# qradiolink/qradiolink

Measured on AMD Instinct MI355X. Metric: IQ MSamples/sec through RX demod chain, higher is better.
Workload: dtype f32

## Files before the change

### qradiolink_amd/csrc/engine.cpp

```cpp
#include "demod.hpp"
#include <cmath>
#include <cstdlib>
#include <memory>
#include <new>

#ifndef QRL_FEC_GATE_US
#define QRL_FEC_GATE_US 30u
#endif
#ifndef QRL_DEV_SKIP
#define QRL_DEV_SKIP 0
#endif

int qrl_demod::flush_fec(bool behind_front_end)
{
    if (!fec_deferred) return QRL_OK;
    fec_deferred = false;
    HIPCHK(hipStreamWaitEvent(fecs, ev_q[fec_pending_slot], 0));
    if (behind_front_end) {
        HIPCHK(hipStreamWaitEvent(fecs, ev_ff, 0));
        launch_fec_gate(QRL_FEC_GATE_US, fecs);
    }
    launch_fec(fec_pending, cfg.batch, fecs);
    HIPCHK(hipEventRecord(ev_fec[fec_pending_slot], fecs));
    return QRL_OK;
// ... 235 lines not shown
        if ((r = fll_lo.upload(to_f2(lo))) || (r = fll_up.upload(to_f2(up)))) return r;
        control_loop_gains((float)(8 * M_PI / 100), fll_alpha, fll_beta);
        fll_maxf = (float)(2 * M_PI * (2.0 / sps_eff));
        if ((r = fll_st.alloc(B))) return r;
        if ((r = tanh_tab.upload(tanh_table())) || (r = qp_st.alloc(B))) return r;
        control_loop_gains((float)(2 * M_PI / 200), c2_alpha, c2_beta);
    } else if (fam == F_QPSK) {
        if ((r = tanh_tab.upload(tanh_table())) || (r = qp_st.alloc(B))) return r;
        control_loop_gains((float)(M_PI / 200 / sps_eff), c1_alpha, c1_beta);
        control_loop_gains((float)(qpsk_fll ? M_PI / 200 : M_PI / 400), c2_alpha, c2_beta);
        if (qpsk_fll) {
            std::vector<std::complex<float>> lo, up;
            fll_band_edge_taps((float)sps_eff, 0.35f, 32, lo, up);
            if ((r = fll_lo.upload(to_f2(lo))) || (r = fll_up.upload(to_f2(up)))) return r;
            control_loop_gains((float)(2 * M_PI / 100), fll_alpha, fll_beta);
            fll_maxf = (float)(2 * M_PI * (2.0 / sps_eff));
            if ((r = fll_st.alloc(B))) return r;
        }
        const float symbol_rate = (float)target / (float)sps_eff;
        const float dev = 200.0f / symbol_rate;
        clock_loop_gains((float)(2 * M_PI / (symbol_rate / 10)), 1.0f, 0.2869f, ss_alpha, ss_beta);
        ss_maxp = (float)sps_eff + dev; ss_minp = (float)sps_eff - dev;
        const float ang = (float)(-3 * M_PI / 4);
        qp_rot = make_float2((float)std::cos((double)ang), (float)std::sin((double)ang));
    } else {
        const std::vector<float> sf = low_pass(1, target, target / sps_eff, target / sps_eff, WIN_HAMMING);
        symf_nt = (int)sf.size();
        if ((r = symf_taps.upload(sf))) return r;
        demod_gain = (float)(sps_eff / (M_PI / 2));
        clock_loop_gains((float)(2 * M_PI / 200.0f), 1.0f, 0.2869f, ss_alpha, ss_beta);
        ss_maxp = (float)sps_eff + 0.05f; ss_minp = (float)sps_eff - 0.05f;
    }
    if ((r = ss_st.alloc(B)) || (r = fec_st.alloc((size_t)B * 2)) || (r = counts_scratch.alloc((size_t)B * 4))) return r;
    if (loops_family() && (r = qp_snap.alloc((size_t)B * 2))) return r;
    if ((fam == F_ANALOG && (r = an.build(*this, mx.n2))) || (fam == F_DSSS && (r = ds.build(*this, mx.n2)))) return r;
    return init_state();
}

int qrl_demod::process(const void* iq, size_t stride, size_t n, const qrl_demod_out* out, int fmt)
{
    if (fmt == IN_SC16 && !fe.used)
        return qrl_set_error(QRL_ERR_ARG, "qrl_demod_process_sc16: int16 input needs the device-rate front end (device_samp_rate >= 2000000); this handle runs at 1 Msps");
    if (n > cfg.max_chunk) return qrl_set_error(QRL_ERR_TOO_BIG, "n exceeds max_chunk");
    if (fmt == IN_SC16) {
        if (!sc16_rows_ok("qrl_demod_process_sc16", iq, stride)) return QRL_ERR_ARG;
    } else if ((reinterpret_cast<uintptr_t>(iq) & 15u) || (stride & 1u)) return qrl_set_error(QRL_ERR_ARG, "iq must be 16-byte aligned, stride even");
    const int B = cfg.batch;
    uint32_t* counts = (out && out->counts) ? out->counts : counts_scratch.p;
    hipStream_t cs = overlap ? tail : stream;
    const int slot = (int)(call_no & 1);
    if (overlap) {
        if (tail2_valid[slot]) HIPCHK(hipStreamWaitEvent(stream, ev_tail2[slot], 0));
    } else {
        HIPCHK(hipMemsetAsync(counts, 0, (size_t)B * 4 * sizeof(uint32_t), stream));
    }
    if (loops_family() && q_valid[slot]) HIPCHK(hipStreamWaitEvent(stream, ev_q[slot], 0));
    if (grouped && q_valid[slot ^ 1]) HIPCHK(hipStreamWaitEvent(stream, ev_q[slot ^ 1], 0));
    if (pre_pending) { HIPCHK(hipStreamWaitEvent(stream, ev_pre, 0)); pre_pending = false; }
    const bool use_pre = pre && input_resident;
    const float2* in = reinterpret_cast<const float2*>(iq);
    const float2* hist_old = hist_flip ? hist_b.p : hist_a.p;
    const PortC fport = filtered_port(out), cport = constellation_port(out);
    float2* hist_new = hist_flip ? hist_a.p : hist_b.p;

    const uint64_t n_in0 = n_in, n_in1 = n_in + n;
    uint64_t n1_0 = n1, n1_1 = n1;
    RingC r2{s2.p, s2_mask}, r2l{s2l.p, s2_mask}, r2f{s2f.p, s2_mask};
    RingF r2d{s2d.p, s2_mask}, r3{s3.p, s2_mask};

    hipEvent_t ev0 = nullptr, ev1 = nullptr;
    if (profiling) {
        HIPCHK(hipEventCreate(&ev0)); HIPCHK(hipEventCreate(&ev1));
        HIPCHK(hipEventRecord(ev0, stream));
    }
    if (fe.used) {
        n1_1 = decim_count(n_in1, 1, fe_decim);
        DecimParams p{};
        p.in = in; p.in_stride = stride; p.n0 = n_in0; p.n = (uint32_t)n;
        p.hist = hist_old; p.hist_len = hist_len;
        p.out = RingC{s1.p, s1_mask}; p.m0 = n1_0; p.m_count = (uint32_t)(n1_1 - n1_0);
        p.taps = fe.taps.p; p.D = fe.D; p.Jpad = fe.c.Jpad;
        p.rot_enable = 1; rot.fill(p);
        p.in_fmt = fmt; p.in_scale = sc16_scale;
        if (use_pre) { p.pre_stream = pre; p.pre_event = ev_pre; }
        if (fe.launch(p, B, stream, use_pre ? slot : 0)) return qrl_set_error(QRL_ERR_HIP, "front-end launch: hipFuncSetAttribute failed");
    }
    if (profiling && fe.used) { HIPCHK(hipEventRecord(ev1, stream)); prof_events.emplace_back(ev0, ev1); }
    const uint64_t src0 = fe.used ? n1_0 : n_in0, src1 = fe.used ? n1_1 : n_in1;
    const uint64_t n2_0 = n2, n2_1 = decim_count(src1, interp, decim);
    if (interp == 1) {
        DecimParams p{};
        input_source(p, in, stride, hist_old, src0, src1);
        p.out = r2; p.m0 = n2_0; p.m_count = (uint32_t)(n2_1 - n2_0);
        p.taps = first.taps.p; p.D = first.D; p.Jpad = first.c.Jpad;
        if (d2f) {
            Dec2FirParams f{};
            f.d = p; f.taps = d2f_taps.p; f.out = RingC{s2f.p, s2_mask};
            f.port = fport.p; f.port_cap = fport.cap; f.counts = counts;
            launch_dec2_fir(f, B, stream);
        } else {
            if (use_pre && !fe.used) { p.pre_stream = pre; p.pre_event = ev_pre; }
            if (first.launch(p, B, stream, use_pre && !fe.used ? slot : 0)) return qrl_set_error(QRL_ERR_HIP, "first-stage launch: hipFuncSetAttribute failed");
        }
    } else {
        ResampParams p{};
        input_source(p, in, stride, hist_old, src0, src1);
        p.out = r2; p.q0 = n2_0; p.q_count = (uint32_t)(n2_1 - n2_0);
        p.taps = rs_taps.p; p.I = interp; p.D = decim; p.Jp = rs_Jp;
        if (fam == F_DMR && !m17) {
            p.port = fport.p; p.port_cap = fport.cap; p.port_counts = counts;
        }
        launch_resamp(p, B, stream);
    }
    if (profiling && !fe.used) { HIPCHK(hipEventRecord(ev1, stream)); prof_events.emplace_back(ev0, ev1); }
    if (scope_out) {
        const uint64_t ns_1 = decim_count(src1, 1, scope_D);
        DecimParams p{};
        input_source(p, in, stride, hist_old, src0, src1);
        p.out = RingC{s_scope.p, scope_mask}; p.m0 = n_scope; p.m_count = (uint32_t)(ns_1 - n_scope);
        p.taps = scope.taps.p; p.D = scope.D; p.Jpad = scope.c.Jpad;
        if (scope.launch(p, B, stream)) return qrl_set_error(QRL_ERR_HIP, "scope launch: hipFuncSetAttribute failed");
        launch_ring_store(RingC{s_scope.p, scope_mask}, n_scope, (uint32_t)(ns_1 - n_scope), scope_out, scope_cap, scope_counts, B, stream);
        n_scope = ns_1;
    }
    {
        HistParams h{};
        h.in = in; h.in_stride = stride; h.n0 = n_in0; h.n = (uint32_t)n;
        h.hist_old = hist_old; h.hist_new = hist_new; h.hist_len = hist_len;
        h.rot_enable = 1; rot.fill(h);
        h.in_fmt = fmt; h.in_scale = sc16_scale;
        if (pre) { HIPCHK(hipEventRecord(ev_fe[slot], stream)); fe_valid[slot] = true; }
        if (use_pre) {
            if (fe_valid[slot ^ 1]) HIPCHK(hipStreamWaitEvent(pre, ev_fe[slot ^ 1], 0));
            launch_hist_save(h, B, pre);
            HIPCHK(hipEventRecord(ev_pre, pre));
            pre_pending = true;
        } else launch_hist_save(h, B, stream);
        hist_flip = !hist_flip;
    }
    if (overlap) {
        HIPCHK(hipEventRecord(ev_ff, stream));
        HIPCHK(hipStreamWaitEvent(tail, ev_ff, 0));
        HIPCHK(hipMemsetAsync(counts, 0, (size_t)B * 4 * sizeof(uint32_t), tail));
    }
    const uint32_t c2 = (uint32_t)(n2_1 - n2_0);
    if (fam == F_DSSS || fam == F_ANALOG) {
        if (int rr = fam == F_DSSS ? ds.stages(*this, n2_0, n2_1, out, counts) : an.stages(*this, n2_0, n2_1, out, counts)) return rr;
        HIPCHK(hipGetLastError());
        if (take_launch_error()) return QRL_ERR_HIP;
        n_in = n_in1; n1 = n1_1; n2 = n2_1; ++call_no;
        return QRL_OK;
    }
    RingC filt_in = r2;
    if (fam == F_2FSK || fam == F_BPSK || (fam == F_QPSK && qpsk_fll)) {
        FllParams f{};
        f.in = r2; f.out = r2l; f.q0 = n2_0; f.count = c2; f.st = fll_st.p;
        f.lower = fll_lo.p; f.upper = fll_up.p; f.nt = fam == F_2FSK ? 16 : 32; f.alpha = fll_alpha; f.beta = fll_beta; f.max_freq = fll_maxf;
        f.slim = fll_slim ? 1 : 0;
        if (!(QRL_DEV_SKIP & 1)) launch_fll(f, B, cs);
        filt_in = r2l;
    }
    const bool fused_2fsk = fam == F_2FSK && !fm && filt_nt <= 41 && disc_nt <= 41 && symf_nt <= 25;
    if (fam == F_DMR) {
        RingC dem_in = r2;
        if (m17) {
            FirCcfParams f{};
            f.in = r2; f.out = r2f; f.q0 = n2_0; f.count = c2; f.taps = filt_taps.p; f.nt = filt_nt;
            f.port = fport.p; f.port_cap = fport.cap; f.counts = counts;
            launch_fir_ccf(f, B, cs);
            dem_in = r2f;
        }
        QuadDemodParams q{}; q.in = dem_in; q.out = r2d; q.q0 = n2_0; q.count = c2; q.gain = demod_gain; q.atan_tab = atan_tab.p;
        launch_quad_demod(q, B, cs);
        if (!overlap && tail_pending) { HIPCHK(hipStreamWaitEvent(stream, ev_tail, 0)); tail_pending = false; }
        FirFffParams f{}; f.in = r2d; f.out = r3; f.q0 = n2_0; f.count = c2; f.taps = symf_taps.p; f.nt = symf_nt;
        launch_fir_fff(f, B, cs);
        if (!overlap) { HIPCHK(hipEventRecord(ev_ff, stream)); HIPCHK(hipStreamWaitEvent(tail, ev_ff, 0)); }
    } else if (fused_2fsk) {
        if (!overlap && tail_pending) { HIPCHK(hipStreamWaitEvent(stream, ev_tail, 0)); tail_pending = false; }
        Fsk2FfParams f{};
        f.in = filt_in; f.out = r3; f.q0 = n2_0; f.count = c2;
        f.tf = ff_tf.p; f.nf = fsk2_ff_padded(filt_nt); f.up = ff_up.p; f.lo = ff_lo.p; f.nb = fsk2_ff_padded(disc_nt);
        f.ts = ff_ts.p; f.ns = fsk2_ff_padded(symf_nt);
        f.port = fport.p; f.port_cap = fport.cap; f.counts = counts;
        if (!(QRL_DEV_SKIP & 2)) launch_2fsk_ff(f, B, cs);
        if (!overlap) { HIPCHK(hipEventRecord(ev_ff, stream)); HIPCHK(hipStreamWaitEvent(tail, ev_ff, 0)); }
    } else {
        if (!d2f) {
            FirCcfParams f{};
            f.in = filt_in; f.out = r2f; f.q0 = n2_0; f.count = c2; f.taps = filt_taps.p; f.nt = filt_nt;
            f.port = fport.p; f.port_cap = fport.cap; f.counts = counts;
            launch_fir_ccf(f, B, cs);
        }
        if (fam == F_QPSK || fam == F_BPSK) {
        } else if (fsk4_disc) {
            RingC r2l4{s2l.p, s2_mask}, r2g{s2g.p, s2_mask};
            Disc4fskParams d{}; d.in = r2f; d.out = r2l4; d.q0 = n2_0; d.count = c2; d.taps = disc4_taps.p; d.nt = disc4_nt;
            launch_disc_4fsk(d, B, cs);
            FirCcfParams f{}; f.in = r2l4; f.out = r2g; f.q0 = n2_0; f.count = c2; f.taps = sym4_taps.p; f.nt = sym4_nt;
            launch_fir_ccf(f, B, cs);
        } else if (fam == F_GMSK || fam == F_4FSK || fm) {
            QuadDemodParams q{}; q.in = r2f; q.out = r2d; q.q0 = n2_0; q.count = c2; q.gain = demod_gain; q.atan_tab = atan_tab.p;
            launch_quad_demod(q, B, cs);
        } else {
            Disc2fskParams d{}; d.in = r2f; d.out = r2d; d.q0 = n2_0; d.count = c2; d.up = disc_up.p; d.lo = disc_lo.p; d.nt = disc_nt;
            launch_disc_2fsk(d, B, cs);
        }
        if (fam == F_QPSK || fam == F_BPSK || fsk4_disc) {
        } else {
            if (!overlap && tail_pending) { HIPCHK(hipStreamWaitEvent(stream, ev_tail, 0)); tail_pending = false; }
            FirFffParams f{}; f.in = r2d; f.out = r3; f.q0 = n2_0; f.count = c2; f.taps = symf_taps.p; f.nt = symf_nt;
            launch_fir_fff(f, B, cs);
            if (!overlap) { HIPCHK(hipEventRecord(ev_ff, stream)); HIPCHK(hipStreamWaitEvent(tail, ev_ff, 0)); }
        }
    }
    if (fam == F_QPSK || fam == F_BPSK || fsk4_disc) {
        QpskParams q{};
        q.in = fsk4_disc ? RingC{s2g.p, s2_mask} : r2f; q.np0 = n2_0; q.avail = n2_1; q.soft = RingB{soft.p, soft_mask}; q.st = qp_st.p;
        q.mmse = mmse_tab.p; q.tanh_tab = tanh_tab.p;
        q.c1_alpha = c1_alpha; q.c1_beta = c1_beta; q.c2_alpha = c2_alpha; q.c2_beta = c2_beta;
        q.ss_alpha = ss_alpha; q.ss_beta = ss_beta; q.ss_maxp = ss_maxp; q.ss_minp = ss_minp;
        q.rot = qp_rot; q.soft_mul = 48.0f; q.soft_add = 128.0f;
        if (fsk4_disc) { q.mode = 2; q.soft_mul = 128.0f; }
        if (fam == F_BPSK) {
            q.mode = 1; q.soft_mul = 64.0f;
            const float gain_omega = 0.005f;
            q.cr_gain_omega = gain_omega * gain_omega; q.cr_gain_mu = 0.05f;
            q.cr_omega_mid = (float)sps_eff; q.cr_omega_lim = 0.001f * (float)sps_eff;
        }
        q.port = cport.p; q.port_cap = cport.cap; q.counts = counts;
        q.oo_snap = qp_snap.p + (size_t)slot * B;
        HIPCHK(hipEventRecord(ev_ff, stream));
        HIPCHK(hipStreamWaitEvent(tail, ev_ff, 0));
        if (q_valid[slot]) HIPCHK(hipStreamWaitEvent(tail, ev_fec[slot], 0));
        launch_qpsk_loops(q, B, tail);
        HIPCHK(hipEventRecord(ev_q[slot], tail));
        if (int rf = flush_fec(true)) return rf;
        if (!grouped) HIPCHK(hipStreamWaitEvent(fecs, ev_q[slot], 0));
        FecParams f{};
        f.soft = RingB{soft.p, soft_mask};
        f.avail = q.oo_snap; f.avail_stride = sizeof(uint64_t); f.avail_mul = fam == F_BPSK ? 1 : 2;
        f.st = fec_st.p;
        f.bits_a = out ? out->bits_a : nullptr; f.bits_b = fam == F_BPSK && out ? out->bits_b : nullptr; f.bits_cap = out ? out->bits_cap : 0;
        f.counts = counts; f.branches = fam == F_BPSK ? 2 : 1;
        if (grouped) { fec_pending = f; fec_pending_slot = slot; fec_deferred = true; }
        else {
            launch_fec(f, B, fecs);
            HIPCHK(hipEventRecord(ev_fec[slot], fecs));
        }
        q_valid[slot] = true;
    } else {
        SymSyncParams s{};
        s.in = r3; s.avail = n2_1; s.soft = RingB{soft.p, soft_mask}; s.st = ss_st.p; s.mmse = mmse_tab.p;
        s.alpha = ss_alpha; s.beta = ss_beta; s.maxp = ss_maxp; s.minp = ss_minp;
        s.ted = fam == F_DMR && !m17 ? 0 : 1; s.soft_mul = 128.0f; s.soft_add = 128.0f;
        s.tail_scale = m17 ? 1.0f : 0.9f;
        s.slim = overlap ? 1 : 0;
        s.slicer = fam == F_DMR || fam == F_4FSK ? 1 : 0; s.tail = fam == F_DMR ? 1 : fam == F_4FSK ? 2 : 0;
        s.bits = out ? out->bits_a : nullptr; s.bits_cap = out ? out->bits_cap : 0;
        s.port = cport.p; s.port_cap = cport.cap; s.counts = counts;
        if (!(QRL_DEV_SKIP & 4)) launch_symsync_ff(s, B, tail);
        if (fam == F_DMR && !m17 && dmo_out) {
            DmoParams dp{}; dp.in = r3; dp.q0 = n2_0; dp.count = (uint32_t)(n2_1 - n2_0); dp.st = dmo_st.p; dp.golay = dmo_golay.p;
            dp.out = dmo_out; dp.cap = dmo_cap; dp.counts = dmo_counts;
            launch_dmo_sink(dp, B, tail);
        }
        if (fam == F_DMR) { HIPCHK(hipEventRecord(ev_tail, tail)); tail_pending = true; }
        FecParams f{};
        f.soft = RingB{soft.p, soft_mask}; f.avail = &ss_st.p[0].oo; f.avail_stride = sizeof(SymSyncState); f.avail_mul = fam == F_4FSK ? 2 : 1; f.st = fec_st.p;
        f.bits_a = out ? out->bits_a : nullptr; f.bits_b = out ? out->bits_b : nullptr; f.bits_cap = out ? out->bits_cap : 0;
        f.counts = counts; f.branches = branches;
        if (fam != F_DMR) {
            if (!(QRL_DEV_SKIP & 8)) launch_fec(f, B, tail);
            HIPCHK(hipEventRecord(ev_tail, tail));
            tail_pending = true;
        }
        if (overlap) { HIPCHK(hipEventRecord(ev_tail2[slot], tail)); tail2_valid[slot] = true; }
    }
    HIPCHK(hipGetLastError());
    if (take_launch_error()) return QRL_ERR_HIP;
    n_in = n_in1; n1 = n1_1; n2 = n2_1; ++call_no;
    return QRL_OK;
}

namespace {
struct Mode { int modem_type; qrl_demod::Family fam; int kind; bool m17, lsb; int sps, filter_width, fm; };
const Mode kModes[] = {
    {QRL_MODEM_2FSK2KFM,  qrl_demod::F_2FSK,   0, false, false, 5,   4000,   1},
    {QRL_MODEM_2FSK1KFM,  qrl_demod::F_2FSK,   0, false, false, 10,  2500,   1},
    {QRL_MODEM_2FSK2K,    qrl_demod::F_2FSK,   0, false, false, 5,   4000,   0},
    {QRL_MODEM_2FSK1K,    qrl_demod::F_2FSK,   0, false, false, 10,  2000,   0},
    {QRL_MODEM_2FSK10KFM, qrl_demod::F_2FSK,   0, false, false, 1,   25000,  1},
    {QRL_MODEM_GMSK2K,    qrl_demod::F_GMSK,   0, false, false, 5,   4000,   0},
    {QRL_MODEM_GMSK1K,    qrl_demod::F_GMSK,   0, false, false, 10,  2000,   0},
    {QRL_MODEM_GMSK10K,   qrl_demod::F_GMSK,   0, false, false, 1,   20000,  0},
    {QRL_MODEM_QPSK250K,  qrl_demod::F_QPSK,   0, false, false, 2,   160000, 0},
    {QRL_MODEM_QPSKVIDEO, qrl_demod::F_QPSK,   0, false, false, 2,   160000, 0},
    {QRL_MODEM_QPSK2K,    qrl_demod::F_QPSK,   0, false, false, 125, 1300,   0},
    {QRL_MODEM_QPSK20K,   qrl_demod::F_QPSK,   0, false, false, 25,  6500,   0},
    {QRL_MODEM_4FSK2K,    qrl_demod::F_4FSK,   0, false, false, 5,   4000,   0},
    {QRL_MODEM_4FSK2KFM,  qrl_demod::F_4FSK,   0, false, false, 5,   3000,   1},
    {QRL_MODEM_4FSK1KFM,  qrl_demod::F_4FSK,   0, false, false, 10,  2000,   1},
    {QRL_MODEM_4FSK10KFM, qrl_demod::F_4FSK,   0, false, false, 1,   20000,  1},
    {QRL_MODEM_4FSK100K,  qrl_demod::F_4FSK,   0, false, false, 2,   125000, 1},
    {QRL_MODEM_BPSK1K,    qrl_demod::F_BPSK,   0, false, false, 10,  1300,   0},
    {QRL_MODEM_BPSK2K,    qrl_demod::F_BPSK,   0, false, false, 5,   2400,   0},
    {QRL_MODEM_DMR,       qrl_demod::F_DMR,    0, false, false, 5,   5000,   0},
    {QRL_MODEM_M17,       qrl_demod::F_DMR,    0, true,  false, 125, 9000,   0},
    {QRL_MODEM_BPSK8,     qrl_demod::F_DSSS,   0, false, false, 25,  150,    0},
    {QRL_MODEM_NBFM2500,  qrl_demod::F_ANALOG, 0, false, false, 125, 2500,   0},
    {QRL_MODEM_NBFM5000,  qrl_demod::F_ANALOG, 0, false, false, 125, 5000,   0},
    {QRL_MODEM_AM5000,    qrl_demod::F_ANALOG, 1, false, false, 125, 5000,   0},
    {QRL_MODEM_WBFM,      qrl_demod::F_ANALOG, 2, false, false, 125, 75000,  0},
    {QRL_MODEM_USB2500,   qrl_demod::F_ANALOG, 3, false, false, 125, 2700,   0},
    {QRL_MODEM_LSB2500,   qrl_demod::F_ANALOG, 3, false, true,  125, 2700,   0},
};
}

extern "C" {

const char* qrl_version(void) { return "qrl_hip 0.1 (gfx950)"; }

int qrl_init(int device, qrl_ctx** ctx)
{
    if (!ctx) return QRL_ERR_ARG;
    int count = 0;
    if (hipGetDeviceCount(&count) != hipSuccess || count <= 0) return qrl_set_error(QRL_ERR_NO_DEVICE, "hipGetDeviceCount: no device");
    if (device < 0 || device >= count) return qrl_set_error(QRL_ERR_NO_DEVICE, "device index out of range");
    HIPCHK(hipSetDevice(device));
    hipDeviceProp_t prop;
    HIPCHK(hipGetDeviceProperties(&prop, device));
    if (std::strncmp(prop.gcnArchName, "gfx950", 6) != 0 && std::strncmp(prop.gcnArchName, "gfx94", 5) != 0)
        return qrl_set_error(QRL_ERR_NO_DEVICE, std::string("unsupported architecture ") + prop.gcnArchName);
    *ctx = new (std::nothrow) qrl_ctx{device};
    return *ctx ? QRL_OK : QRL_ERR_NOMEM;
}
void qrl_shutdown(qrl_ctx* ctx) { delete ctx; }

// ... 288 lines not shown
```

### qradiolink_amd/csrc/engine.hpp

```cpp
#pragma once
#include <hip/hip_runtime.h>
#include <stdint.h>
#include <vector>
#include "zero_runs.hpp"
#include "decim_plan.hpp"

namespace qrl {

hipError_t dyn_lds_limit(const void* kernel, int bytes);
bool take_launch_error();

int create_role_stream(hipStream_t* s, int priority, const char* role);

struct RingC { float2* p; uint32_t mask; };
struct RingF { float* p; uint32_t mask; };
struct RingB { uint8_t* p; uint32_t mask; };

template <class Pp>
__device__ __forceinline__ void rot_select(Pp& c, const Pp& p, uint32_t b)
{
    c = p; c.rot_acc = p.rot_acc_s[b]; c.rot_inc = p.rot_inc_s[b]; c.rot_lo = p.rot_lo + (size_t)b * 512;
}
#define ROT_VIEW(T, PS, P, SRC, B) T P##_ps_; if constexpr (PS) rot_select(P##_ps_, SRC, (uint32_t)(B)); const T& P = (PS) ? P##_ps_ : SRC
std::vector<float2> rot_fine_table(uint64_t inc);
void launch_rot_ps_advance(uint64_t* acc, const uint64_t* inc, int B, uint64_t delta, hipStream_t s);
void launch_rot_ps_fill(uint64_t* acc, uint64_t* inc, float2* lo, int B, int set_acc, uint64_t acc0, uint64_t inc0, const float2* lo0, hipStream_t s);

enum { IN_CF32 = 0, IN_SC16 = 1 };
__device__ __forceinline__ float2 sc16_to_f2(uint32_t w, float scale)
{
    return make_float2((float)(int16_t)(w & 0xffffu) * scale, (float)((int32_t)w >> 16) * scale);
}
template <class Pp>
__device__ __forceinline__ float2 in_load(const Pp& P, size_t b, size_t r)
{
    if (P.in_fmt == IN_SC16) return sc16_to_f2(reinterpret_cast<const uint32_t*>(P.in)[b * P.in_stride + r], P.in_scale);
    return P.in[b * P.in_stride + r];
}
template <bool SC, class Pp>
__device__ __forceinline__ float2 in_load_as(const Pp& P, size_t b, size_t r)
{
    if constexpr (SC) return sc16_to_f2(reinterpret_cast<const uint32_t*>(P.in)[b * P.in_stride + r], P.in_scale);
    else return P.in[b * P.in_stride + r];
}

struct Sc16Out { int on; float scale; uint32_t* clip; };

struct DecimParams {
    const float2* in; size_t in_stride;
    RingC in_ring;
    uint64_t n0; uint32_t n;
    const float2* hist; uint32_t hist_len;
    RingC out;
    uint64_t m0; uint32_t m_count;
    const float* taps;
    int D, Jpad;
    int rot_enable; uint64_t rot_acc; uint64_t rot_inc; uint64_t rot_nbase; const float2* rot_lo;
    uint32_t tiles;
    const float* gtab; int S; int nt; uint32_t magic_blk, magic_seg;
    uint32_t tpw, nchunks; int nhi; int dbg;
    int nld;
    int hist_raw;
    uint32_t out_row_mul_m1, out_row_add;
    const float* pl_taps; int pl_J; uint32_t pl_S, pl_nseg, pl_batch; uint64_t pl_m_begin, pl_m_end;
    int pl_E, pl_R; const float* pl_hraw;
    float2* pl_edge; uint32_t pl_edge_stride, pl_edge_cap; uint64_t pl_edge_ms, pl_edge_me;
    hipStream_t pre_stream; hipEvent_t pre_event;
    const uint64_t* rot_acc_s; const uint64_t* rot_inc_s;
    int in_fmt; float in_scale;
};
struct HistParams {
    const float2* in; size_t in_stride; uint64_t n0; uint32_t n;
    const float2* hist_old; float2* hist_new; uint32_t hist_len;
    int rot_enable; uint64_t rot_acc; uint64_t rot_inc; uint64_t rot_nbase; const float2* rot_lo;
    const uint64_t* rot_acc_s; const uint64_t* rot_inc_s;
    int in_fmt; float in_scale;
};
void launch_decim(const DecimParams& p, int batch, int variant, hipStream_t s);
struct Dec2FirParams { DecimParams d; const float* taps; RingC out; float2* port; size_t port_cap; uint32_t* counts; };
bool dec2_fir_supported(int nt1, int D, int nt2);
uint32_t dec2_fir_lookback();
std::vector<float> dec2_fir_table(const std::vector<float>& h1, const std::vector<float>& h2);
void launch_dec2_fir(const Dec2FirParams& p, int batch, hipStream_t s);
void launch_hist_save(const HistParams& p, int batch, hipStream_t s);
int launch_decim_mfma(const DecimParams& p, int batch, hipStream_t s);
void decim_mfma_prof_read(unsigned long long* out8);
void decim_mfma_prof_enable(int on);
std::vector<float> decim_pl_layout(const std::vector<float>& h, int D);
int launch_decim_pl(const DecimParams& p, int batch, hipStream_t s);
std::vector<float> decim_pm_layout(const std::vector<float>& h, int D);
int launch_decim_pm(const DecimParams& p, int batch, hipStream_t s);

struct ResampParams {
    const float2* in; size_t in_stride; uint64_t n0; uint32_t n;
    int in_fmt;
    const float2* hist; uint32_t hist_len;
    float in_scale;
    RingC in_ring;
    RingC out;
    uint64_t q0; uint32_t q_count;
    const float* taps;
    int I, D, Jp;
    int rot_enable; uint64_t rot_acc; uint64_t rot_inc; uint64_t rot_nbase; const float2* rot_lo;
    float2* port; size_t port_cap; uint32_t* port_counts;
    const uint64_t* rot_acc_s; const uint64_t* rot_inc_s;
};
void launch_resamp(const ResampParams& p, int batch, hipStream_t s);

struct FirCcfParams { RingC in; RingC out; uint64_t q0; uint32_t count; const float* taps; int nt;
                      float2* port; size_t port_cap; uint32_t* counts; };
struct FirFffParams { RingF in; RingF out; uint64_t q0; uint32_t count; const float* taps; int nt; };
struct QuadDemodParams { RingC in; RingF out; uint64_t q0; uint32_t count; float gain; const float* atan_tab;
                         RingF out2; float gain2;
                         int16_t* s16; size_t s16_cap; float s16_level, s16_scale; uint32_t* s16_counts; };
struct Disc2fskParams { RingC in; RingF out; uint64_t q0; uint32_t count; const float2* up; const float2* lo; int nt; };
struct Disc4fskParams { RingC in; RingC out; uint64_t q0; uint32_t count; const float2* taps; int nt; };
void launch_disc_4fsk(const Disc4fskParams& p, int batch, hipStream_t s);
struct Fsk2FfParams { RingC in; RingF out; uint64_t q0; uint32_t count;
                      const float* tf; int nf; const float2* up; const float2* lo; int nb; const float* ts; int ns;
                      float2* port; size_t port_cap; uint32_t* counts; };
void launch_2fsk_ff(const Fsk2FfParams& p, int batch, hipStream_t s);
int fsk2_ff_padded(int n);
void launch_fir_ccf(const FirCcfParams& p, int batch, hipStream_t s);
void launch_fir_fff(const FirFffParams& p, int batch, hipStream_t s);
void launch_quad_demod(const QuadDemodParams& p, int batch, hipStream_t s);
void launch_disc_2fsk(const Disc2fskParams& p, int batch, hipStream_t s);

struct FllState { float phase, freq; float2 dl[32]; };
struct FllParams { RingC in; RingC out; uint64_t q0; uint32_t count; FllState* st;
                   const float2* lower; const float2* upper; int nt; float alpha, beta, max_freq;
                   int slim; };
void launch_fll(const FllParams& p, int batch, hipStream_t s);

struct SymSyncState { uint64_t ii; uint64_t oo; float mu, avg, inst; float x0, x1, x2, d0, d1, d2; };
struct SymSyncParams {
    RingF in; uint64_t avail;
    RingB soft;
    SymSyncState* st;
    const float* mmse;
    float alpha, beta, maxp, minp;
    int ted; float soft_mul, soft_add;
    int slicer;
    float tail_scale;
    int tail;
    uint8_t* bits; size_t bits_cap;
    float2* port; size_t port_cap; uint32_t* counts;
    int slim;
};
void launch_symsync_ff(const SymSyncParams& p, int batch, hipStream_t s);

struct QpskState {
    uint64_t ii, oo;
    float gain;
    float c1_phase, c1_freq;
    float mu, avg, inst;
    float2 x0, x1, x2, d0, d1, d2;
    float c2_phase, c2_freq;
    float2 dprev;
    float2 hist[16];
};
struct QpskParams {
    RingC in; uint64_t np0, avail;
    RingB soft; QpskState* st;
    const float* mmse; const float* tanh_tab;
    float c1_alpha, c1_beta, c2_alpha, c2_beta;
    float ss_alpha, ss_beta, ss_maxp, ss_minp;
    float2 rot; float soft_mul, soft_add;
    int mode;
    float cr_gain_omega, cr_gain_mu, cr_omega_mid, cr_omega_lim;
    float2* port; size_t port_cap; uint32_t* counts;
    uint64_t* oo_snap;
};
void launch_qpsk_loops(const QpskParams& p, int batch, hipStream_t s);

struct FecState { uint64_t consumed; uint32_t start_state; uint32_t last_bits; };
struct FecParams {
    RingB soft; const uint64_t* avail; size_t avail_stride; uint32_t avail_mul;
    FecState* st;
    uint8_t* bits_a; uint8_t* bits_b; size_t bits_cap; uint32_t* counts;
    int branches;
};
void launch_fec(const FecParams& p, int batch, hipStream_t s);
void launch_fec_gate(unsigned us, hipStream_t s);

struct DmoState {
    uint32_t bitBuffer[5];
    uint16_t syncPtr, startPtr, endPtr, pad0;
    float maxCorr, centre[4], threshold[4];
    uint8_t averagePtr, syncCount, state, control, n, colorCode, pad1[2];
};
struct DmoParams { RingF in; uint64_t q0; uint32_t count; DmoState* st; const uint32_t* golay; uint8_t* out; uint32_t cap; uint32_t* counts; };
void launch_dmo_sink(const DmoParams& p, int batch, hipStream_t s);
std::vector<uint32_t> golay1987_table();

struct DeframeState { uint32_t reg, found, idx, pad; };
struct DeframeParams {
    const uint8_t* bits; size_t stride; uint32_t n;
    const uint32_t* counts; size_t count_stride;
    int type; uint32_t buf_len; DeframeState* st;
    uint8_t* out; size_t out_cap; uint32_t* out_counts;
};
void launch_deframe(const DeframeParams& p, int batch, hipStream_t s);
struct FrameSyncState { uint32_t reg, found, idx, ftype, modem_sync, pad[3]; };
struct FrameSyncParams {
    const uint8_t* bits; size_t stride; uint32_t n; const uint32_t* counts; size_t count_stride;
    int cls; uint32_t bit_buf_len, frame_length;
    FrameSyncState* st; uint8_t* bitbuf; size_t bitbuf_stride;
    uint8_t* out; size_t out_cap; uint32_t* out_counts;
    uint32_t* activity;
};
void launch_framesync(const FrameSyncParams& p, int batch, hipStream_t s);

struct ChanParams {
    const float2* in; size_t in_stride; uint64_t n0; uint32_t n;
    int in_fmt;
    const float2* hist; uint32_t hist_len;
    float in_scale;
    RingC out; uint64_t m0; uint32_t m_count;
    const float* taps; const float2* twiddle;
    int M, J, c_first, c_count;
    int legacy;
    uint32_t row_cpd; size_t out_pitch;
};
struct F2sParams { RingF in; uint64_t q0; uint32_t count; float level, scale; int16_t* out; size_t cap; uint32_t* counts; };
struct RssiParams { RingC in; uint64_t j0; uint32_t count; float calibration; float* out; size_t cap; uint32_t* counts; };
void launch_rssi_tag(const RssiParams& p, int batch, hipStream_t s);
struct ChanTailParams {
    RingC in;
    const float2* lin; size_t lin_pitch; uint64_t lin_base; uint32_t lin_n; const float2* hist; uint32_t hist_len;
    uint64_t q0; uint32_t count;
    const float* tab_a; const float* tab_b; const float* tab_e;
    const float* atan_tab;
    float gain, gain2, level, scale;
    int16_t* s16; size_t s16_cap; uint32_t* s16_counts;
    RingF out_sym;
    float* rssi; size_t rssi_cap; uint32_t* rssi_counts; float rssi_cal; uint64_t tag0; uint32_t ntags;
};
void launch_chan_tail(const ChanTailParams& p, int streams, hipStream_t s);
bool chan_tail_supported(int rs_I, int rs_D, int rs_Jp, int filt_nt, int rrc_nt);
std::vector<float> chan_tail_tables(int which, const float* taps);
uint32_t chan_tail_lookback();
void launch_pfb_chan(const ChanParams& p, int batch, hipStream_t s);
void launch_ring_store(RingC in, uint64_t q0, uint32_t count, float2* out, size_t cap, uint32_t* counts, int rows, hipStream_t s);
void launch_ring_load(const float2* in, size_t pitch, RingC out, uint64_t q0, uint32_t count, int rows, hipStream_t s);
void launch_f2s(const F2sParams& p, int batch, hipStream_t s);
size_t chan_lds_bytes(int M, int J);
struct S2fInParams { const int16_t* in; size_t in_stride; RingF out; uint64_t q0; uint32_t count; float scale, level; };
struct SynthParams {
    RingC in; int nch;
    int port_chan[16];
    uint64_t blk0; uint32_t nblk;
    const float* taps; const float2* twiddle; int M, J;
    float level, bb_gain;
    float2* out; size_t out_stride, out_cap;
    Sc16Out sc;
};
void launch_s2f_in(const S2fInParams& p, int streams, hipStream_t s);
void launch_scale_c(RingC r, uint64_t q0, uint32_t count, float k, int streams, hipStream_t s);
void launch_zero_runs(RingC r, const ZeroRun* runs, uint32_t nruns, uint64_t lo, uint64_t hi, hipStream_t s);
void launch_pfb_synth(const SynthParams& p, int batch, hipStream_t s);
void launch_ring_store_sc16(RingC in, uint64_t q0, uint32_t count, uint32_t* out, size_t out_stride, Sc16Out sc, int rows, hipStream_t s);
size_t synth_lds_bytes(int M, int J);

struct TxState { uint32_t sr, enc, prev, pad; };
struct TxBitsParams {
    const uint8_t* bytes; size_t stride; uint32_t nbytes; uint32_t L;
    uint8_t tl_pow[6][8];
    int mode;
    TxState* st; RingB sym; uint64_t s0;
};
struct TxInterpParams {
    RingB sym; uint64_t n0; uint32_t count;
    const float* taps; int nt; int interp; float2 table[4]; float amp, bb_gain;
    float2* out; size_t out_stride;
    Sc16Out sc;
};
struct TxShapeParams { RingB sym; RingF out; uint64_t n0; uint32_t count; int sps; const float* taps; int nt;
                       int levels; float scale; };
struct TxFmParams { RingF in; RingC out; uint64_t n0; uint32_t count; float k, amp; float* phase; };
struct TxInterpCParams { RingC in; uint64_t n0; uint32_t count; const float* taps; int nt; int interp; float2* out; size_t out_stride;
                         int decim; RingC out_ring; Sc16Out sc; };
constexpr int kTxMfmaPhases = 32, kTxMfmaLags = 210;
struct TxInterpMfmaParams { RingC in; uint64_t n0; uint32_t n1; const float* taps; int interp; uint32_t cpw;
                            float2* out; size_t out_stride; Sc16Out sc; };
void launch_tx_interp_mfma(const TxInterpMfmaParams& p, int batch, hipStream_t s);
// ... 93 lines not shown
```

Baseline: 541,300.

## Fuse 2FSK FLL with filter/discriminator/symbol FIR into one pipelined kernel

Adds a fused kernel for the 2FSK path in which dedicated FLL waves run the frequency-locked loop window by window and write the corrected samples into LDS. FIR waves in the same block consume those windows through the channel filter, band-edge discriminator and symbol filter, with block barriers pipelining the two roles. This removes the separate FLL launch and the global-memory round trip of the FLL output, writing back only the history the next call needs. In exchange the kernel is large and LDS-heavy, and its serial FLL waves set the pace. It is used only when the tap counts match fixed geometry and the slim FLL is off.

```diff
diff --git a/qradiolink_amd/csrc/engine.cpp b/qradiolink_amd/csrc/engine.cpp
--- a/qradiolink_amd/csrc/engine.cpp
+++ b/qradiolink_amd/csrc/engine.cpp
@@ -411,15 +411,17 @@
         return QRL_OK;
     }
     RingC filt_in = r2;
+    const bool fused_2fsk = fam == F_2FSK && !fm && filt_nt <= 41 && disc_nt <= 41 && symf_nt <= 25;
+    const bool tail_fused = fsk2_tail_eligible(fused_2fsk, 16, fsk2_ff_padded(filt_nt), fsk2_ff_padded(disc_nt), fsk2_ff_padded(symf_nt), fll_slim);
+    FllParams fllp{};
     if (fam == F_2FSK || fam == F_BPSK || (fam == F_QPSK && qpsk_fll)) {
-        FllParams f{};
+        FllParams& f = fllp;
         f.in = r2; f.out = r2l; f.q0 = n2_0; f.count = c2; f.st = fll_st.p;
         f.lower = fll_lo.p; f.upper = fll_up.p; f.nt = fam == F_2FSK ? 16 : 32; f.alpha = fll_alpha; f.beta = fll_beta; f.max_freq = fll_maxf;
         f.slim = fll_slim ? 1 : 0;
-        if (!(QRL_DEV_SKIP & 1)) launch_fll(f, B, cs);
+        if (!(QRL_DEV_SKIP & 1) && !tail_fused) launch_fll(f, B, cs);
         filt_in = r2l;
     }
-    const bool fused_2fsk = fam == F_2FSK && !fm && filt_nt <= 41 && disc_nt <= 41 && symf_nt <= 25;
     if (fam == F_DMR) {
         RingC dem_in = r2;
         if (m17) {
@@ -442,7 +444,10 @@
         f.tf = ff_tf.p; f.nf = fsk2_ff_padded(filt_nt); f.up = ff_up.p; f.lo = ff_lo.p; f.nb = fsk2_ff_padded(disc_nt);
         f.ts = ff_ts.p; f.ns = fsk2_ff_padded(symf_nt);
         f.port = fport.p; f.port_cap = fport.cap; f.counts = counts;
-        if (!(QRL_DEV_SKIP & 2)) launch_2fsk_ff(f, B, cs);
+        if (tail_fused) {
+            Fsk2TailParams t{}; t.fll = fllp; t.ff = f;
+            if (!(QRL_DEV_SKIP & 3)) launch_2fsk_tail(t, B, cs);
+        } else if (!(QRL_DEV_SKIP & 2)) launch_2fsk_ff(f, B, cs);
         if (!overlap) { HIPCHK(hipEventRecord(ev_ff, stream)); HIPCHK(hipStreamWaitEvent(tail, ev_ff, 0)); }
     } else {
         if (!d2f) {
diff --git a/qradiolink_amd/csrc/engine.hpp b/qradiolink_amd/csrc/engine.hpp
--- a/qradiolink_amd/csrc/engine.hpp
+++ b/qradiolink_amd/csrc/engine.hpp
@@ -4,6 +4,7 @@
 #include <vector>
 #include "zero_runs.hpp"
 #include "decim_plan.hpp"
+#include "fsk2_tail_geo.hpp"
 
 namespace qrl {
 
@@ -131,6 +132,9 @@
                    const float2* lower; const float2* upper; int nt; float alpha, beta, max_freq;
                    int slim; };
 void launch_fll(const FllParams& p, int batch, hipStream_t s);
+struct Fsk2TailParams { FllParams fll; Fsk2FfParams ff; };
+void launch_2fsk_tail(const Fsk2TailParams& p, int batch, hipStream_t s);
+size_t fsk2_tail_lds_bytes();
 
 struct SymSyncState { uint64_t ii; uint64_t oo; float mu, avg, inst; float x0, x1, x2, d0, d1, d2; };
 struct SymSyncParams {
diff --git a/qradiolink_amd/csrc/fsk2_tail_geo.hpp b/qradiolink_amd/csrc/fsk2_tail_geo.hpp
--- /dev/null
+++ b/qradiolink_amd/csrc/fsk2_tail_geo.hpp
@@ -0,0 +1,51 @@
+#pragma once
+#include <stddef.h>
+#include <stdint.h>
+
+namespace qrl {
+
+struct Fsk2TailGeo {
+    static constexpr int W = 16, WW = W / 4;
+    static constexpr int FLL_NT = 16;
+    static constexpr int QF = 11, QB = 11, QS = 7;
+    static constexpr int HF = 4 * (QF - 1), HB = 4 * (QB - 1), HS = 4 * (QS - 1);
+    static constexpr int KEEP = HF + HB + HS;
+    static constexpr int YW = 20, FW = 16, DW = 16;
+    static constexpr int YWIN = YW / WW, FWIN = FW / WW;
+    static constexpr int YP = 4 * YW + 4, FP = 4 * FW + 4, DP = 4 * DW + 4;
+    static constexpr int XP = W + 1;
+    static constexpr int FIRST = -4;
+    static constexpr int LOAD0 = -7;
+    static constexpr int KEEP_WIN = 8;
+
+    static_assert(KEEP == 104, "history of the three filters");
+    static_assert(YW >= 2 * WW + QF + 1 && YW % WW == 0, "y ring: a window being written, one being read, QF words of history and the zero-tap word");
+    static_assert(FW >= WW + QB + 1 && FW % WW == 0 && DW >= WW + QS + 1 && DW % WW == 0, "f / d rings");
+    static_assert(-LOAD0 * W >= KEEP && (-FIRST + 0) * WW + QF <= -LOAD0 * WW, "the fetch covers what the first FIR window reads");
+    static_assert(-FIRST * W >= HB + HS && 2 * W >= HS, "stage 1 from q0 - 64, stage 2 from q0 - 32 <= q0 - 24");
+    static_assert(KEEP_WIN * W >= KEEP + W - 1, "the windows written back hold the last KEEP samples for any count");
+    static_assert(YWIN >= -FIRST + 1, "windows FIRST .. -1 and window 0 do not share a slot: the FLL starts beside the FIR window -1");
+
+    static constexpr int threads(int ns) { return 4 * ns + 64 * (ns / 16); }
+    static constexpr size_t off_y(int) { return 0; }
+    static constexpr size_t off_f(int ns) { return off_y(ns) + (size_t)ns * YP * 8; }
+    static constexpr size_t off_x(int ns) { return off_f(ns) + (size_t)ns * FP * 8; }
+    static constexpr size_t off_dump(int ns) { return off_x(ns) + (size_t)ns * XP * 8; }
+    static constexpr size_t off_d(int ns) { return off_dump(ns) + (size_t)ns * 4 * 8; }
+    static constexpr size_t off_taps(int ns) { return off_d(ns) + (size_t)ns * DP * 4; }
+    static constexpr size_t lds_bytes(int ns) { return off_taps(ns) + (size_t)(4 * QF + 8 * QB + 4 * QS) * 4; }
+
+    static constexpr int nwin(uint32_t count) { return (int)((count + (uint32_t)W - 1) / (uint32_t)W); }
+    static constexpr int slot_y(int j) { return ((j % YWIN) + YWIN) % YWIN; }
+    static constexpr int slot_f(int j) { return ((j % FWIN) + FWIN) % FWIN; }
+    static constexpr int first_keep_window(uint32_t count) { return nwin(count) > KEEP_WIN ? nwin(count) - KEEP_WIN : 0; }
+    static constexpr int barriers(uint32_t count) { return 1 + (nwin(count) - (FIRST + 1) + 1); }
+};
+
+inline bool fsk2_tail_eligible(bool fsk2_non_fm, int fll_nt, int nf, int nb, int ns, bool fll_slim)
+{
+    return fsk2_non_fm && !fll_slim && fll_nt == Fsk2TailGeo::FLL_NT && (nf - 1) / 4 + 1 == Fsk2TailGeo::QF && (nb - 1) / 4 + 1 == Fsk2TailGeo::QB &&
+           (ns - 1) / 4 + 1 == Fsk2TailGeo::QS;
+}
+
+}
diff --git a/qradiolink_amd/csrc/kernels_2fsk_tail.hip b/qradiolink_amd/csrc/kernels_2fsk_tail.hip
--- /dev/null
+++ b/qradiolink_amd/csrc/kernels_2fsk_tail.hip
@@ -0,0 +1,293 @@
+#include "devmath.hpp"
+#include "engine.hpp"
+#include "fsk2_tail_geo.hpp"
+
+namespace qrl {
+
+template <int CTRL> __device__ __forceinline__ float tl_dpp_quad(float v)
+{
+    return __builtin_bit_cast(float, __builtin_amdgcn_mov_dpp(__builtin_bit_cast(int, v), CTRL, 0xF, 0xF, true));
+}
+__device__ __forceinline__ void tl_wave_sync()
+{
+    __builtin_amdgcn_fence(__ATOMIC_RELEASE, "wavefront");
+    __builtin_amdgcn_wave_barrier();
+    __builtin_amdgcn_fence(__ATOMIC_ACQUIRE, "wavefront");
+}
+
+template <int NW, int NQ, typename TapT, typename ItemT, typename Fma>
+__device__ __forceinline__ void tl_window4(const ItemT* __restrict__ rows, int w, const TapT* __restrict__ taps, Fma&& fma4)
+{
+    ItemT cur[4], nxt[4];
+#pragma unroll
+    for (int s = 0; s < 4; ++s) cur[s] = rows[s * NW + w];
+#pragma unroll
+    for (int q = 0; q < NQ; ++q) {
+        w = (w == 0 ? NW : w) - 1;
+#pragma unroll
+        for (int s = 0; s < 4; ++s) nxt[s] = rows[s * NW + w];
+        const TapT h0 = taps[4 * q], h1 = taps[4 * q + 1], h2 = taps[4 * q + 2], h3 = taps[4 * q + 3];
+        fma4(h0, cur[0], cur[1], cur[2], cur[3]);
+        fma4(h1, nxt[3], cur[0], cur[1], cur[2]);
+        fma4(h2, nxt[2], nxt[3], cur[0], cur[1]);
+        fma4(h3, nxt[1], nxt[2], nxt[3], cur[0]);
+#pragma unroll
+        for (int s = 0; s < 4; ++s) cur[s] = nxt[s];
+    }
+}
+
+template <int NS>
+__global__ __launch_bounds__(Fsk2TailGeo::threads(NS)) void k_2fsk_tail(const Fsk2TailParams P, int batch)
+{
+    using G = Fsk2TailGeo;
+    constexpr int TH = G::threads(NS), NFLL = NS / 16;
+    constexpr int NT = G::FLL_NT, GL = NT / 4, W = G::W;
+    constexpr int YW = G::YW, FW = G::FW, DW = G::DW, YP = G::YP, FP = G::FP, DP = G::DP, XP = G::XP;
+    static_assert(NS % 16 == 0 && TH <= 1024, "whole waves of 16 streams");
+    extern __shared__ __align__(16) unsigned char tl_smem[];
+    float2* const Y = reinterpret_cast<float2*>(tl_smem + G::off_y(NS));
+    float2* const F = reinterpret_cast<float2*>(tl_smem + G::off_f(NS));
+    float2* const X = reinterpret_cast<float2*>(tl_smem + G::off_x(NS));
+    float2* const dump = reinterpret_cast<float2*>(tl_smem + G::off_dump(NS));
+    float* const D = reinterpret_cast<float*>(tl_smem + G::off_d(NS));
+
+    const int tid = threadIdx.x, wv = tid >> 6, lane = tid & 63;
+    const bool is_fll = wv < NFLL;
+    const int b0 = blockIdx.x * NS;
+    const int nstreams = min(NS, batch - b0);
+    const uint32_t count = P.fll.count;
+    const int nwin = G::nwin(count);
+    const uint64_t q0 = P.fll.q0;
+
+    for (int i = tid; i < (int)(G::off_taps(NS) / 4); i += TH) reinterpret_cast<uint32_t*>(tl_smem)[i] = 0u;
+    float* const T = reinterpret_cast<float*>(tl_smem + G::off_taps(NS));
+    for (int i = tid; i < 4 * G::QF; i += TH) T[i] = P.ff.tf[i];
+    for (int i = tid; i < 4 * G::QB; i += TH) reinterpret_cast<float2*>(T + 4 * G::QF)[i] = P.ff.up[i];
+    for (int i = tid; i < 4 * G::QS; i += TH) T[4 * G::QF + 8 * G::QB + i] = P.ff.ts[i];
+    const float* const tap_f = T; const float2* const tap_b = reinterpret_cast<const float2*>(T + 4 * G::QF); const float* const tap_s = T + 4 * G::QF + 8 * G::QB;
+    __syncthreads();
+
+    const int sl = is_fll ? tid >> 2 : 0, g = tid & 3;
+    const bool fll_active = is_fll && b0 + sl < batch;
+    float phase = 0.f, freq = 0.f;
+    float2 dl[GL], hu[GL], hl[GL];
+    constexpr int NPT = W * 16 / 64;
+    float2 pre[NPT];
+#pragma unroll
+    for (int t = 0; t < GL; ++t) { dl[t] = make_float2(0.f, 0.f); hu[t] = hl[t] = make_float2(0.f, 0.f); }
+#pragma unroll
+    for (int i = 0; i < NPT; ++i) pre[i] = make_float2(0.f, 0.f);
+    auto preload = [&](uint32_t c0) {
+#pragma unroll
+        for (int i = 0; i < NPT; ++i) {
+            const int s = min(16 * wv + (lane >> 4) + 4 * i, nstreams - 1), k = lane & 15;
+            const int64_t a = (int64_t)(q0 + c0 + k) - NT;
+            const float2 v = P.fll.in.p[(size_t)(b0 + s) * (P.fll.in.mask + 1u) + ((uint32_t)a & P.fll.in.mask)];
+            pre[i] = a >= 0 ? v : make_float2(0.f, 0.f);
+        }
+    };
+    const int fs = is_fll ? 0 : 16 * (wv - NFLL) + (lane >> 2), ft = lane & 3;
+    const int fb = b0 + fs;
+    const bool fir_active = !is_fll && fb < batch;
+    float2* const Ys = Y + fs * YP;
+    float2* const Fs = F + fs * FP;
+    float* const Ds = D + fs * DP;
+    const bool al4 = (q0 & 3u) == 0;
+    float hold[4] = {0.f, 0.f, 0.f, 0.f};
+    auto fetch_y = [&](int pj, float2 (&v)[4]) {
+#pragma unroll
+        for (int r = 0; r < 4; ++r) {
+            const int off = W * pj + 4 * ft + r;
+            const int64_t a = (int64_t)q0 + off;
+            const float2 x = P.ff.in.p[(size_t)(b0 + min(fs, nstreams - 1)) * (P.ff.in.mask + 1u) + ((uint32_t)a & P.ff.in.mask)];
+            v[r] = (a >= 0 && off >= -G::KEEP && fir_active) ? x : make_float2(0.f, 0.f);
+        }
+    };
+    auto put_y = [&](int pj, const float2 (&v)[4]) {
+#pragma unroll
+        for (int r = 0; r < 4; ++r) Ys[r * YW + 4 * G::slot_y(pj) + ft] = v[r];
+    };
+    auto store_r3 = [&](int jw, const float (&v)[4]) {
+        const uint32_t t0 = (uint32_t)(W * jw + 4 * ft);
+        if (!fir_active || t0 >= count) return;
+        float* const row = P.ff.out.p + (size_t)fb * (P.ff.out.mask + 1u);
+        const uint64_t n = q0 + t0;
+        if (al4 && t0 + 3u < count) *reinterpret_cast<float4*>(row + ((uint32_t)n & P.ff.out.mask)) = make_float4(v[0], v[1], v[2], v[3]);
+        else {
+#pragma unroll
+            for (int r = 0; r < 4; ++r) if (t0 + r < count) row[(uint32_t)(n + r) & P.ff.out.mask] = v[r];
+        }
+    };
+
+    if (is_fll) {
+        if (fll_active) {
+            const FllState& s = P.fll.st[b0 + sl];
+            phase = s.phase; freq = s.freq;
+#pragma unroll
+            for (int t = 0; t < GL; ++t) dl[t] = s.dl[g * GL + t];
+        }
+#pragma unroll
+        for (int t = 0; t < GL; ++t) { hu[t] = P.fll.upper[g * GL + t]; hl[t] = P.fll.lower[g * GL + t]; }
+        preload(0);
+        int ys_w = 0;
+        for (int j = G::FIRST + 1; j <= nwin; ++j) {
+            if (j >= 0 && j < nwin) {
+                const uint32_t c0 = (uint32_t)(W * j);
+                const int len = min((uint32_t)W, count - c0);
+#pragma unroll
+                for (int i = 0; i < NPT; ++i) X[(16 * wv + (lane >> 4) + 4 * i) * XP + (lane & 15)] = pre[i];
+                tl_wave_sync();
+                if (j + 1 < nwin) preload(c0 + W);
+                if (fll_active) {
+                    const float2* const xw = X + sl * XP;
+                    float2* const yr = Y + sl * YP + 4 * ys_w;
+                    for (int k = 0; k < len; ++k) {
+                        const float2 x = xw[k];
+                        const float2 nco = sincos_rad(phase);
+                        float2 carry;
+                        carry.x = tl_dpp_quad<0x90>(dl[GL - 1].x);
+                        carry.y = tl_dpp_quad<0x90>(dl[GL - 1].y);
+#pragma unroll
+                        for (int t = GL - 1; t > 0; --t) dl[t] = dl[t - 1];
+                        float ur = 0.f, ui = 0.f, lr = 0.f, li = 0.f;
+#pragma unroll
+                        for (int t = GL - 1; t >= 1; --t) {
+                            const float2 v = dl[t];
+                            ur = fmaf(hu[t].x, v.x, ur); ur = fmaf(-hu[t].y, v.y, ur);
+                            ui = fmaf(hu[t].x, v.y, ui); ui = fmaf(hu[t].y, v.x, ui);
+                            lr = fmaf(hl[t].x, v.x, lr); lr = fmaf(-hl[t].y, v.y, lr);
+                            li = fmaf(hl[t].x, v.y, li); li = fmaf(hl[t].y, v.x, li);
+                        }
+                        const float2 y = cmul(x, nco);
+                        *(g == 0 ? &yr[(k & 3) * YW + (k >> 2)] : &dump[tid]) = y;
+                        dl[0] = g == 0 ? y : carry;
+                        {
+                            const float2 v = dl[0];
+                            ur = fmaf(hu[0].x, v.x, ur); ur = fmaf(-hu[0].y, v.y, ur);
+                            ui = fmaf(hu[0].x, v.y, ui); ui = fmaf(hu[0].y, v.x, ui);
+                            lr = fmaf(hl[0].x, v.x, lr); lr = fmaf(-hl[0].y, v.y, lr);
+                            li = fmaf(hl[0].x, v.y, li); li = fmaf(hl[0].y, v.x, li);
+                        }
+                        ur = ur + tl_dpp_quad<0xB1>(ur); ui = ui + tl_dpp_quad<0xB1>(ui); lr = lr + tl_dpp_quad<0xB1>(lr); li = li + tl_dpp_quad<0xB1>(li);
+                        ur = ur + tl_dpp_quad<0x4E>(ur); ui = ui + tl_dpp_quad<0x4E>(ui); lr = lr + tl_dpp_quad<0x4E>(lr); li = li + tl_dpp_quad<0x4E>(li);
+                        const float error = (lr * lr + li * li) - (ur * ur + ui * ui);
+                        freq = freq + P.fll.beta * error;
+                        phase = phase + freq + P.fll.alpha * error;
+                        phase = phase_wrap(phase);
+                        freq = __builtin_fminf(__builtin_fmaxf(freq, -P.fll.max_freq), P.fll.max_freq);
+                    }
+                }
+                ys_w = ys_w == G::YWIN - 1 ? 0 : ys_w + 1;
+            }
+            __syncthreads();
+        }
+        if (fll_active) {
+            FllState& s = P.fll.st[b0 + sl];
+            if (g == 0) { s.phase = phase; s.freq = freq; }
+#pragma unroll
+            for (int t = 0; t < GL; ++t) s.dl[g * GL + t] = dl[t];
+        }
+    } else {
+        float2 v[4][4];
+#pragma unroll
+        for (int i = 0; i < 4; ++i) fetch_y(G::LOAD0 + i, v[i]);
+#pragma unroll
+        for (int i = 0; i < 4; ++i) put_y(G::LOAD0 + i, v[i]);
+        static_assert(G::LOAD0 + 3 == G::FIRST, "windows LOAD0 .. FIRST in front of the loop, one more per prologue trip");
+        int ys_r = G::slot_y(G::FIRST), fs_r = G::slot_f(G::FIRST);
+        for (int j = G::FIRST + 1; j <= nwin; ++j) {
+            const int jw = j - 1;
+            const int64_t n0 = (int64_t)q0 + W * jw + 4 * ft;
+            const uint32_t t0 = (uint32_t)(W * jw + 4 * ft);
+            float2 nv[4];
+            if (jw < -1) fetch_y(jw + 1, nv);
+            if (jw >= 0) {
+                if (jw == 0 && ft == 0 && fir_active && P.ff.counts) P.ff.counts[fb * 4 + 0] = count;
+                if (jw >= nwin - G::KEEP_WIN && fir_active) {
+#pragma unroll
+                    for (int r = 0; r < 4; ++r)
+                        if (t0 + r < count) P.ff.in.p[(size_t)fb * (P.ff.in.mask + 1u) + ((uint32_t)(n0 + r) & P.ff.in.mask)] = Ys[r * YW + 4 * ys_r + ft];
+                }
+            }
+            {
+                float2 a[4] = {{0.f, 0.f}, {0.f, 0.f}, {0.f, 0.f}, {0.f, 0.f}};
+                tl_window4<YW, G::QF>(Ys, 4 * ys_r + ft, tap_f,
+                                      [&](float h, const float2& x0, const float2& x1, const float2& x2, const float2& x3) {
+                                          a[0].x = fmaf(h, x0.x, a[0].x); a[0].y = fmaf(h, x0.y, a[0].y);
+                                          a[1].x = fmaf(h, x1.x, a[1].x); a[1].y = fmaf(h, x1.y, a[1].y);
+                                          a[2].x = fmaf(h, x2.x, a[2].x); a[2].y = fmaf(h, x2.y, a[2].y);
+                                          a[3].x = fmaf(h, x3.x, a[3].x); a[3].y = fmaf(h, x3.y, a[3].y);
+                                      });
+#pragma unroll
+                for (int r = 0; r < 4; ++r) {
+                    if (n0 + r < 0) a[r] = make_float2(0.f, 0.f);
+                    Fs[r * FW + 4 * fs_r + ft] = a[r];
+                }
+                if (jw >= 0 && fir_active && P.ff.port) {
+#pragma unroll
+                    for (int r = 0; r < 4; ++r)
+                        if (t0 + r < count && t0 + r < P.ff.port_cap) P.ff.port[(size_t)fb * P.ff.port_cap + t0 + r] = a[r];
+                }
+            }
+            tl_wave_sync();
+            if (jw >= -2) {
+                float ar[4] = {0.f, 0.f, 0.f, 0.f}, ai[4] = {0.f, 0.f, 0.f, 0.f}, br[4] = {0.f, 0.f, 0.f, 0.f}, bi[4] = {0.f, 0.f, 0.f, 0.f};
+                tl_window4<FW, G::QB>(Fs, 4 * fs_r + ft, tap_b,
+                                      [&](const float2 h, const float2& x0, const float2& x1, const float2& x2, const float2& x3) {
+                                          const float2 xs[4] = {x0, x1, x2, x3};
+#pragma unroll
+                                          for (int r = 0; r < 4; ++r) {
+                                              ar[r] = fmaf(h.x, xs[r].x, ar[r]); ai[r] = fmaf(h.x, xs[r].y, ai[r]);
+                                              br[r] = fmaf(h.y, xs[r].x, br[r]); bi[r] = fmaf(h.y, xs[r].y, bi[r]);
+                                          }
+                                      });
+#pragma unroll
+                for (int r = 0; r < 4; ++r) {
+                    const float ur = ar[r] - bi[r], ui = ai[r] + br[r], lr = ar[r] + bi[r], li = ai[r] - br[r];
+                    const float mu = sqrtf(ur * ur + ui * ui);
+                    const float ml = sqrtf(lr * lr + li * li);
+                    float v = mu / ml;
+                    if (!(v >= 0.0f)) v = 0.0f;
+                    if (v > 2.0f) v = 2.0f;
+                    Ds[r * DW + 4 * fs_r + ft] = (n0 + r < 0) ? 0.f : v + (-1.0f);
+                }
+                tl_wave_sync();
+            }
+            if (jw >= 0) {
+                float a[4] = {0.f, 0.f, 0.f, 0.f};
+                tl_window4<DW, G::QS>(Ds, 4 * fs_r + ft, tap_s,
+                                      [&](float h, float x0, float x1, float x2, float x3) {
+                                          a[0] = fmaf(h, x0, a[0]); a[1] = fmaf(h, x1, a[1]); a[2] = fmaf(h, x2, a[2]); a[3] = fmaf(h, x3, a[3]);
+                                      });
+                if ((jw & 1) == 0 && jw != nwin - 1) {
+#pragma unroll
+                    for (int r = 0; r < 4; ++r) hold[r] = a[r];
+                } else {
+                    if (jw & 1) store_r3(jw - 1, hold);
+                    store_r3(jw, a);
+                }
+            }
+            if (jw < -1) put_y(jw + 1, nv);
+            ys_r = ys_r == G::YWIN - 1 ? 0 : ys_r + 1;
+            fs_r = (fs_r + 1) & (G::FWIN - 1);
+            __syncthreads();
+        }
+    }
+}
+
+#ifndef QRL_TAIL_NS
+#define QRL_TAIL_NS 64
+#endif
+size_t fsk2_tail_lds_bytes() { return Fsk2TailGeo::lds_bytes(QRL_TAIL_NS); }
+
+void launch_2fsk_tail(const Fsk2TailParams& p, int batch, hipStream_t s)
+{
+    if (!p.fll.count) return;
+    constexpr int NS = QRL_TAIL_NS;
+    const auto k = k_2fsk_tail<NS>;
+    const size_t lds = Fsk2TailGeo::lds_bytes(NS);
+    if (dyn_lds_limit(reinterpret_cast<const void*>(k), (int)lds) != hipSuccess) return;
+    hipLaunchKernelGGL(k, dim3((batch + NS - 1) / NS), dim3(Fsk2TailGeo::threads(NS)), lds, s, p, batch);
+}
+
+}
```

Result: faster. 551,600 (median of 6 runs) (+1.9%).
